# jmloveyj/ros_navigation

Measured on AMD Instinct MI355X. Metric: replan cycles/sec (HIMM+VFH++A*) on 4096x4096 grid, higher is better.
Workload: dtype int32; 1 GPU; full replan loop on 4096x4096 f32 grid (res 0.05 m); one step = one turn of the 20-stage A* pipeline = 20 passes of [100032-ray HIMM batch + fused compose -> 256 VFH+ poses -> 256 grid-A* queries (one launch)]; 30% rectangle obstacles (seed 2); 4 ray batches / pose sets / query sets in rotation; cycles_per_pass=256, rays_per_pass=100032, rotating_input_sets=4, astar_queries_checked=15360, astar_queries_answered=15360, astar_bucket_width=128000, astar_pipeline_depth=20, parallelism=query-sharded x1, full=False

## Files before the change

ros_navigation_amd/csrc/astar.hip:

```cpp
#include "engine.hpp"

#include <algorithm>
#include <cfloat>
#include <cmath>
#include <cstdlib>
#include <cstring>
#include <chrono>
#include <thread>
#include <vector>

using namespace rna;

namespace {

constexpr int COST_D = 1414;

struct HostTrace {
  bool on = getenv("RNA_HOST_TRACE") != nullptr;
  double us[8] = {};
  long n = 0, queries = 0;
  std::chrono::steady_clock::time_point t;
  void start() { if (on) t = std::chrono::steady_clock::now(); }
  void lap(int k) {
    if (!on) return;
// ... 166 lines not shown
  static const bool nowait = getenv("RNA_ASTAR_NOWAIT") != nullptr;
  static const int per_look = getenv("RNA_ASTAR_QUERIES_PER_LOOK") ? std::max(1, atoi(getenv("RNA_ASTAR_QUERIES_PER_LOOK"))) : 3;
  int slot = -1;
  for (int spin = 0; slot < 0; ++spin) {
    int oldest = 0;
    for (int d = 0; d < a.depth; ++d) {
      if (a.stage[d].seq < a.stage[oldest].seq) oldest = d;
      if (!a.stage[d].busy && (slot < 0 || a.stage[d].seq < a.stage[slot].seq)) slot = d;
    }
    if (slot < 0) {
      int order[AstarDevice::MAX_DEPTH], nb = 0;
      for (int d = 0; d < a.depth; ++d) if (a.stage[d].busy) order[nb++] = d;
      std::sort(order, order + nb, [&](int x, int y) { return a.stage[x].seq < a.stage[y].seq; });
      const int ask = (spin & 7) == 7 ? nb : std::min(nb, per_look);
      for (int k = 0; k < ask && slot < 0; ++k) {
        const int d = order[k];
        g_trace.queries += 1;
        if (hipEventQuery(a.stage[d].done) != hipSuccess) { (void)hipGetLastError(); continue; }
        bool sent = false;
        RNA_TRY(stage_settled(e, d, &sent));
        if (sent) continue;
        a.stage[d].busy = false;
        slot = d;
        if (g_trace.on && g_stage.armed[d]) {
          float f = 0;
          if (hipEventElapsedTime(&f, g_stage.a[d], g_stage.c[d]) == hipSuccess) {
            g_stage.gpu_ms += f; g_stage.n += 1;
            g_stage.host_busy_ms += std::chrono::duration<double, std::milli>(std::chrono::steady_clock::now() - g_stage.t_enq[d]).count();
          }
          g_stage.armed[d] = false;
        }
      }
    }
    if (slot >= 0) break;
    if (nowait) { slot = oldest; break; }
    static const int wait_us = getenv("RNA_ASTAR_WAIT_US") ? atoi(getenv("RNA_ASTAR_WAIT_US")) : 50;
    if (spin >= 2 && wait_us > 0) std::this_thread::sleep_for(std::chrono::microseconds(wait_us));
    else std::this_thread::yield();
  }
  g_trace.lap(0);
  const unsigned long long prev = a.launches + 1 >= (unsigned long long)a.ring_n ? a.launches + 1 - (unsigned long long)a.ring_n : 0;
  for (int d = 0; prev > 0 && d < a.depth; ++d)
    if (a.stage[d].busy && a.stage[d].seq == prev) RNA_TRY(stage_wait(e, d));
  *slot_out = slot;
  return RNA_OK;
}

int launch_chunk(rna_engine* e, const rna_astar_query* q_dev, int n, int32_t* paths_dev, int max_len,
                 rna_astar_result* res_dev, int* slot_out) {
  AstarDevice& a = e->astar;
  const bool pipelined = a.depth > 1;
  int slot = 0, r = -1;
  g_trace.start();
  if (pipelined) RNA_TRY(pick_stage(e, &slot));
  g_trace.lap(1);
  if (!pipelined && stage_pending(a, 0)) RNA_TRY(stage_wait(e, 0));
  AstarStage& s = a.stage[slot];
  hipStream_t search = stage_stream(e, slot), prep = search;
  if (pipelined) {
    if (s.busy) RNA_HIP(e, hipStreamWaitEvent(search, s.done, 0));
    if (g_trace.on) {
      if (!g_stage.a[slot]) { (void)hipEventCreate(&g_stage.a[slot]); (void)hipEventCreate(&g_stage.c[slot]); }
      (void)hipEventRecord(g_stage.a[slot], search);
      g_stage.t_enq[slot] = std::chrono::steady_clock::now();
    }
    r = (int)(a.launches % (unsigned long long)a.ring_n);
    RNA_TRY(side_stream(e, &prep));
    RNA_HIP(e, hipEventRecord(a.ev_init, e->stream));
    RNA_HIP(e, hipStreamWaitEvent(prep, a.ev_init, 0));
    if (a.ring[r].used) RNA_HIP(e, hipStreamWaitEvent(prep, a.ring[r].free, 0));
  }
  RNA_TRY(tsa_snapshot(e, slot, r, prep));
  if (pipelined) {
    RNA_HIP(e, hipEventRecord(s.snap_done, prep));
    s.snap_pending = true;
  }
  RNA_TRY(tsa_order(e, slot, r, prep, q_dev, n));
  if (pipelined) {
    RNA_HIP(e, hipEventRecord(a.ev_prep, prep));
    RNA_HIP(e, hipStreamWaitEvent(search, a.ev_prep, 0));
  }
  if (s.retry_flag) *s.retry_flag = 0;
  RNA_TRY(tsa_search(e, slot, r, search, q_dev, n, paths_dev, max_len, res_dev));
  if (s.retry_armed) RNA_HIP(e, hipMemcpyAsync(s.retry_flag, tsa_retry_count(e, slot), sizeof(int), hipMemcpyDeviceToHost, search));
  if (pipelined) {
    RNA_HIP(e, hipEventRecord(a.ring[r].free, search));
    a.ring[r].used = true;
    if (g_trace.on) { (void)hipEventRecord(g_stage.c[slot], search); g_stage.armed[slot] = true; }
  }
  g_trace.lap(2);
  if (pipelined) {
    RNA_HIP(e, hipEventRecord(s.done, search));
    s.busy = true;
  }
  a.launches += 1;
  s.seq = a.launches;
  a.last_queries = q_dev; a.last_results = res_dev; a.last_n = n; a.last_slot = slot;
  if (slot_out) *slot_out = slot;
  g_trace.lap(3);
  if (pipelined) g_trace.n += 1;
  return RNA_OK;
}

}

namespace rna {
#ifdef RNA_TSA_STATS
void tsa_stats_dump();
#endif
int astar_settle(rna_engine* e) {
  AstarDevice& a = e->astar;
  for (int d = 0; d < a.depth && d < AstarDevice::MAX_DEPTH; ++d)
    if (stage_pending(a, d)) RNA_TRY(stage_wait(e, d));
  return RNA_OK;
}
int astar_release(rna_engine* e) {
  AstarDevice& a = e->astar;
  (void)sync_all(e);
  stage_trace_dump();
  g_trace.dump();
#ifdef RNA_TSA_STATS
  tsa_stats_dump();
#endif
  for (AstarStage& s : a.stage) free_stage(s);
  if (a.ev_init) { (void)hipEventDestroy(a.ev_init); a.ev_init = nullptr; }
  if (a.ev_prep) { (void)hipEventDestroy(a.ev_prep); a.ev_prep = nullptr; }
  for (AstarRingEntry& r : a.ring) {
    if (r.free) (void)hipEventDestroy(r.free);
    r = AstarRingEntry{};
  }
  dev_free(&a.ring_mem);
  a.ring_n = 0;
  if (a.retry_flag) { (void)hipHostFree(a.retry_flag); a.retry_flag = nullptr; }
  dev_free(&a.queries_dev); dev_free(&a.results_dev); dev_free(&a.paths_dev);
  a.paths_cap = 0;
  a.last_queries = nullptr; a.last_results = nullptr; a.last_n = 0;
  return RNA_OK;
}
}

extern "C" int rna_astar_configure(rna_engine* e, int max_queries, int queue_capacity, int bucket_width) {
  if (!e || max_queries < 0 || queue_capacity < 0 || bucket_width < 0) return RNA_EINVAL;
  if (bucket_width != 0 && bucket_width < 2 * COST_D) return fail(e, RNA_EINVAL, "bucket_width must be >= 2828");
  RNA_ENTER(e);
  RNA_HIP(e, hipStreamSynchronize(e->stream));
  AstarDevice& a = e->astar;
  if (max_queries || queue_capacity) astar_release(e);
  if (const char* d = getenv("RNA_ASTAR_PIPELINE")) {
    const int dd = atoi(d);
    if (dd >= 1 && dd != a.depth) { astar_release(e); a.depth = dd; }
  }
  if (max_queries) a.max_queries = max_queries;
  if (bucket_width) a.bucket_width = bucket_width;
  return RNA_OK;
}

extern "C" int rna_astar_set_pipeline_depth(rna_engine* e, int depth) {
  if (!e || depth < 1 || depth > AstarDevice::MAX_DEPTH) return RNA_EINVAL;
  RNA_ENTER(e);
  if (depth != e->astar.depth) {
    astar_release(e);
    e->astar.depth = depth;
  }
  char advice[448];
  if (rna_hw_queue_advice(depth, advice, sizeof(advice))) e->err = advice;
  return RNA_OK;
}
// ... 108 lines not shown
```

ros_navigation_amd/csrc/astar_tile.hip:

```cpp
#include "engine.hpp"
#include <algorithm>
#include <cstring>
#include <vector>

using namespace rna;

namespace rna {

constexpr int TI = 64, TJ = 16;
constexpr int TILE_WORDS = TI * TJ;
constexpr int AUX_WORDS = 64;
constexpr int MASK_STRIDE = TILE_WORDS + 32 + 128;
constexpr int TSA_WAVES = 8;
constexpr int TSA_WAVES_PER_EU = 8;
constexpr int TSA_HPASS = 4;
constexpr int TSA_IDLE_SLEEP = 4;
constexpr int TSA_PRIO_FIRST = 0;
constexpr int TSA_BT_PRIO = 3;
constexpr int TSA_SCOPE = __HIP_MEMORY_SCOPE_AGENT;
constexpr int TSA_MAX_TILE_WORDS = 2048;
constexpr int COST_S = 1000, COST_D = 1414;
constexpr int INF = 0x7fffffff;
constexpr int KU = 0x40000000;
constexpr int SCR_CNT = 84 + 192 + 48 + 64;
// ... 868 lines not shown
        cp[0] = make_uint4((unsigned)pp0, (unsigned)pp1, (unsigned)pp2, (unsigned)pp3);
        cp[1] = make_uint4((unsigned)pp4, (unsigned)pp5, (unsigned)pp6, (unsigned)pp7);
        cp[2] = make_uint4((unsigned)pp8, (unsigned)pp9, (unsigned)pp10, (unsigned)pp11);
        cp[3] = make_uint4((unsigned)pp12, (unsigned)pp13, (unsigned)pp14, (unsigned)pp15);
      }
      __builtin_amdgcn_wave_barrier();
      const int xl_ = lane & 31;
      const bool xr_ = lane >= 32;
      const int v_ = (xl_ >= 1 && xl_ <= TJ) ? (int)scr[276 + (lane & 32) + xl_ - 1] : 0;
      const int xv = (int)scr[84 + 128 + lane];
      const unsigned eb_ = scr[84 + 192 + 48 + lane];
      const int vs_ = v_ & -(int)((eb_ >> (xr_ ? 4 : 3)) & 1u), vu_ = v_ & -(int)((eb_ >> (xr_ ? 2 : 0)) & 1u), vd_ = v_ & -(int)((eb_ >> (xr_ ? 7 : 5)) & 1u);
      const int from_below_ = lane_p1(vu_) + nD, from_above_ = lane_m1(vd_) + nD;
      const int ux_ = max3i(vs_ + nS, from_below_, from_above_);
      const bool imp = (xl_ <= TJ + 1) & (ux_ > xv);
      const unsigned long long im = __builtin_amdgcn_ballot_w64(imp);
      const unsigned lo = (unsigned)im, hi = (unsigned)(im >> 32);
      colw = (lo & 1u) | ((lo >> 12) & 32u) | ((hi & 1u) << 2) | ((hi >> 10) & 128u) | ((lo & 0x1fffeu) ? 8u : 0u) | ((hi & 0x1fffeu) ? 16u : 0u);
      if (im) {
        const int hX_ = tsa_octile24(xr_ ? i0 + TI : i0 - 1, j0 + xl_ - 1, gi, gj);
        wave_halves_max_i32(imp ? ux_ - hX_ : (int)0x80000000, kfW, kfE);
      }
      __builtin_amdgcn_wave_barrier();
    }
    const unsigned am = colw | (wakeN ? 2u : 0u) | (wakeS ? 64u : 0u);
    const unsigned wm = am & (unsigned)__builtin_amdgcn_ballot_w64(nb_t >= 0);
    if (wm) {
      asm volatile("s_waitcnt vmcnt(0)" ::: "memory");
      int kf = __builtin_amdgcn_inverse_ballot_w64(0x29ull) ? kfW : kfE;
      kf = __builtin_amdgcn_inverse_ballot_w64(0x02ull) ? kfN : kf;
      kf = __builtin_amdgcn_inverse_ballot_w64(0x40ull) ? kfS : kf;
      int key = (key_base - kf) >> key_shift;
      key = key < 0 ? 0 : (key > TSA_NCLS - 1 ? TSA_NCLS - 1 : key);
      TSA_T(t_w1);
      sch.wake8(__builtin_amdgcn_inverse_ballot_w64((unsigned long long)wm), nb_t, (unsigned)key, lane, spare);
      TSA_T(t_w2);
      TSA_ACC(3, t_w1, t_w2);
      TSA_CNT(13, 1);
    }
  }
  asm volatile("; TSA_MARK job_end");
  TSA_T(t_d);
  TSA_ACC(2, t_c, t_d);
  TSA_ACC(6, t_w0, t_d);
  if (lane_in == 0) { atomicAdd(&scr[SCR_CNT], (unsigned)__builtin_popcount(rowchg)); atomicAdd(&scr[SCR_CNT + 1], 1u); }
  }
tsa_job_done:
  asm volatile("s_waitcnt vmcnt(0)" ::: "memory");
  {
    int t_f = t_in;
    asm volatile("" : "+s"(t_f));
    const int again = sch.finish(t_f, lane_in, spare, scr + SCR_CNT);
    if (!again) break;
    first_w = again >> 1;
    sticky_w = 1;
    TSA_CNT(7, 1);
    TSA_CNT(22, 1);
  }
  }
#undef TSA_ROW_CHANGED
#undef TSA_H
}

struct TsaLaunch {
  int rows, cols, tiles_i, tiles_j, s0, s1;
  const rna_astar_query* queries;
  TsaStage S;
  int bucket_width;
  int prio_first;
  int retry, n;
  int* retry_count;
  int* retry_list;
  int retry_base;
  TsaStage S2;
  int32_t* paths;
  int max_path_len;
  int32_t* rev_all;
  int rev_cap;
  rna_astar_result* results;
};
constexpr int TSA_FOUND = -1000;

constexpr int BW = TI + 2;
__device__ __forceinline__ void tsa_backtrace_wave(const TsaLaunch& A, const TsaStage& S, const int sl, const int q, const rna_astar_result r,
                                                   const int lane, unsigned* s_tile, unsigned char* s_mask) {
  const int rows = A.rows, cols = A.cols, tiles_i = A.tiles_i, tiles_j = A.tiles_j;
  const int ncell = rows * cols, ntile = tiles_i * tiles_j;
  const unsigned* tmap = S.tmap + (size_t)sl * ntile;
  const size_t page_base = (size_t)sl * ((size_t)S.cap + 1);
  const int start = tsa_unwrap_lin(A.queries[q].start, rows, cols, A.s0, A.s1);
  const int goal = tsa_unwrap_lin(A.queries[q].goal, rows, cols, A.s0, A.s1);
  const int si = start % rows, sj = start / rows;
  int ci = goal % rows, cj = goal / rows;
  int* rev = A.rev_all + (size_t)q * A.rev_cap;
  const int k = lane & 7;
  const int wk = (k == 1 || k == 3 || k == 4 || k == 6) ? COST_S : COST_D;
  const int di = kdi_of(k), dj = kdj_of(k);
  const int off = di + dj * BW;
  int len = 0;
  bool ok = true, done = false;
#ifdef RNA_TSA_STATS
  unsigned long long bt_loads = 0, bt_load_ticks = 0;
#endif
  while (ok && !done) {
#ifdef RNA_TSA_STATS
    const unsigned long long t_l0 = wall_clock64();
#endif
    const int ti = ci >> 6, tj = cj >> 4;
    const int t = tj * tiles_i + ti;
    unsigned pgl = 0u;
    {
      const int nti = lane < 8 ? ti + di : ti, ntj = lane < 8 ? tj + dj : tj;
      if (lane < 9 && nti >= 0 && ntj >= 0 && nti < tiles_i && ntj < tiles_j) pgl = ld_l2(&tmap[ntj * tiles_i + nti]);
    }
    auto gpage = [&](int src) -> size_t {
      const unsigned lp = (unsigned)__shfl((int)pgl, src);
      return page_base + lp;
    };
    {
      const int xl = lane & 31;
      const bool xr = lane >= 32;
      const unsigned* pown = S.pages + (gpage(8) << 10);
      const unsigned top = ld_l2(&S.pages[(gpage(1) << 10) + (TJ - 1) * TI + lane]);
      const unsigned bot = ld_l2(&S.pages[(gpage(6) << 10) + lane]);
      const int xdir = xl == 0 ? (xr ? 2 : 0) : (xl <= TJ ? (xr ? 4 : 3) : (xr ? 7 : 5));
      const int xrow = xl == 0 ? TJ - 1 : (xl <= TJ ? xl - 1 : 0);
      const size_t gpx = gpage(xdir);
      unsigned X = 0u;
      if (xl <= TJ + 1) X = ld_l2(&S.paux[gpx * AUX_WORDS + (xr ? 0 : 16) + xrow]);
      unsigned tv[TJ];
#pragma unroll
      for (int b = 0; b < TJ; ++b) tv[b] = ld_l2(&pown[b * TI + lane]);
      const uint4 mv = *reinterpret_cast<const uint4*>(S.nbr_tm + (size_t)t * MASK_STRIDE + lane * 16);
      __builtin_amdgcn_wave_barrier();
      s_tile[lane + 1] = top;
      s_tile[(TJ + 1) * BW + lane + 1] = bot;
      if (xl <= TJ + 1) s_tile[xl * BW + (xr ? TI + 1 : 0)] = X;
#pragma unroll
      for (int b = 0; b < TJ; ++b) s_tile[(b + 1) * BW + lane + 1] = tv[b];
      *reinterpret_cast<uint4*>(&s_mask[lane * 16]) = mv;
    }
    asm volatile("s_waitcnt vmcnt(0) lgkmcnt(0)" ::: "memory");
    __builtin_amdgcn_wave_barrier();
#ifdef RNA_TSA_STATS
    bt_loads += 1; bt_load_ticks += wall_clock64() - t_l0;
#endif
    int il = ci & (TI - 1), jl = cj & (TJ - 1);
    unsigned uc = s_tile[(jl + 1) * BW + il + 1];
    for (;;) {
      if (lane == 0 && len < A.rev_cap) rev[len] = cj * rows + ci;
      ++len;
      if (ci == si && cj == sj) { done = true; break; }
      if (len > ncell || uc == 0u) { ok = false; break; }
      const unsigned mc = s_mask[il * 16 + jl];
      const unsigned un = s_tile[(jl + 1) * BW + il + 1 + off];
      const bool hit = (lane < 8) & (((mc >> k) & 1u) != 0u) & (un != 0u) & (un == uc + (unsigned)wk);
      const unsigned long long m = __ballot(hit);
      if (!m) { ok = false; break; }
      const int src = __builtin_ctz((unsigned)m);
      uc = (unsigned)__builtin_amdgcn_readlane((int)un, src);
      const int sdi = kdi_of(src), sdj = kdj_of(src);
      ci += sdi; cj += sdj; il += sdi; jl += sdj;
      if (il < 0 || jl < 0 || il >= TI || jl >= TJ) break;
    }
  }
#ifdef RNA_TSA_STATS
  if (lane == 0) { atomicAdd(&g_tsa_stat[27], bt_loads); atomicAdd(&g_tsa_stat[28], bt_load_ticks); atomicAdd(&g_tsa_stat[29], (unsigned long long)len); }
#endif
  if (!ok) {
    if (lane == 0) A.results[q] = rna_astar_result{1, 0, INF, r.expanded, r.rounds, r.buckets};
    return;
  }
  if (len > A.max_path_len || len > A.rev_cap) {
    if (lane == 0) A.results[q] = rna_astar_result{3, len, r.cost, r.expanded, r.rounds, r.buckets};
    return;
  }
  asm volatile("s_waitcnt vmcnt(0)" ::: "memory");
  __builtin_amdgcn_wave_barrier();
  int32_t* path = A.paths + (size_t)q * A.max_path_len;
  for (int i = lane; i < len; i += 64) path[i] = tsa_buffer_lin(rev[len - 1 - i], rows, cols, A.s0, A.s1);
  if (lane == 0) A.results[q] = rna_astar_result{0, len, r.cost, r.expanded, r.rounds, r.buckets};
}

template <int WAVES, bool RETRY>
__global__ void __launch_bounds__(WAVES * 64) __attribute__((amdgpu_waves_per_eu(TSA_WAVES_PER_EU, TSA_WAVES_PER_EU))) tsa_search_kernel(const TsaLaunch A) {
  constexpr int TSA_THREADS = WAVES * 64;
  __shared__ __attribute__((aligned(16))) unsigned s_scr[WAVES][SCR_WORDS];
  extern __shared__ unsigned s_dyn[];
  __shared__ __attribute__((aligned(16))) unsigned s_node[TSA_NP];
  __shared__ __attribute__((aligned(16))) unsigned s_head[TSA_NCLS];
  __shared__ unsigned s_bm[TSA_BMW];
  __shared__ unsigned s_qc[TSA_QC];
  __shared__ int s_best, s_state, s_bucket, s_bucket0, s_jobs_done, s_jobs_noop, s_jobs_sticky, s_expanded, s_nalloc, s_any;
  __shared__ int s_count, s_spill, s_idle, s_open_left, s_open_pos, s_reruns;

  __shared__ int s_q, s_rank;
  if (!RETRY) {
    if (threadIdx.x == 0) { const int k = atomicAdd(A.S.ticket, 1); s_rank = k; s_q = A.S.perm[k]; }
  } else {
    if (threadIdx.x == 0) { s_q = A.retry_list[A.retry_base + (int)blockIdx.x]; s_rank = 1 << 30; }
  }
  __syncthreads();
  const int q = __builtin_amdgcn_readfirstlane(s_q);
  if (q < 0) return;
  if (RETRY && threadIdx.x == 0) A.S2.ticket[8 + blockIdx.x] = q;
  const TsaStage& S = RETRY ? A.S2 : A.S;
  const int sl = RETRY ? (int)blockIdx.x : q;
  if (__builtin_amdgcn_readfirstlane(s_rank) < A.prio_first) __builtin_amdgcn_s_setprio(3);
  const int tid = threadIdx.x, lane = tid & 63, wv = __builtin_amdgcn_readfirstlane(tid >> 6);
#ifdef RNA_TSA_STATS
  const unsigned long long t_kernel0 = wall_clock64();
#endif
  const int rows = A.rows, cols = A.cols, tiles_i = A.tiles_i, tiles_j = A.tiles_j;
  rna_astar_query qu = A.queries[q];
  const int ncell = rows * cols;
  const int ntile = tiles_i * tiles_j;
  const int nt_words = (ntile + 31) >> 5;
  unsigned* const s_st2 = s_dyn;
  unsigned* const s_open = s_dyn + 2 * nt_words;
  unsigned* const s_far = s_dyn + 3 * nt_words;
  rna_astar_result* const results = A.results;

  const bool valid = qu.start >= 0 && qu.goal >= 0 && qu.start < ncell && qu.goal < ncell;
  if (!valid) {
    if (tid == 0) results[q] = rna_astar_result{2, 0, INF, 0, 0, 0};
    return;
  }
  qu.start = tsa_unwrap_lin(qu.start, rows, cols, A.s0, A.s1);
  qu.goal = tsa_unwrap_lin(qu.goal, rows, cols, A.s0, A.s1);
  const int si = qu.start % rows, sj = qu.start / rows;
  const int gi = qu.goal % rows, gj = qu.goal / rows;

  TsaCtx C;
  C.rows = rows; C.cols = cols; C.tiles_i = tiles_i; C.tiles_j = tiles_j;
  C.tiles_magic = tiles_i > 1 ? (unsigned)(0x100000000ull / (unsigned)tiles_i) + 1u : 0u;
  C.pages = S.pages + (((size_t)sl * ((size_t)S.cap + 1)) << 10);
  C.paux = S.paux + (size_t)sl * ((size_t)S.cap + 1) * AUX_WORDS;
  C.tmap = S.tmap + (size_t)sl * ntile;
  C.owner = S.owner + (size_t)sl * (S.cap + 1);
  C.cap = S.cap;
  C.nalloc = &s_nalloc;
  C.nbr_tm = S.nbr_tm;
  C.gi = gi; C.gj = gj;
  C.ts = tile_of(si, sj, tiles_i); C.sa = si & (TI - 1); C.sb = sj & (TJ - 1);
  C.tg = tile_of(gi, gj, tiles_i); C.ga = gi & (TI - 1); C.gb = gj & (TJ - 1);

  for (int w = tid; w < 4 * nt_words; w += TSA_THREADS) s_dyn[w] = 0u;
  for (int w = tid; w < TSA_NCLS; w += TSA_THREADS) s_head[w] = 0xffffu;
  for (int w = tid; w < TSA_BMW; w += TSA_THREADS) s_bm[w] = 0xffffffffu;
  for (int w = tid; w < TSA_QC; w += TSA_THREADS) s_qc[w] = 0xffffffffu;
  if (lane >= 48) s_scr[wv][68 + lane - 48] = 0u;
  if (lane < 4) s_scr[wv][SCR_CNT + lane] = 0u;
  {
    const unsigned ms = C.nbr_tm[(size_t)C.ts * MASK_STRIDE + C.sa * 16 + C.sb], mg = C.nbr_tm[(size_t)C.tg * MASK_STRIDE + C.ga * 16 + C.gb];
    if (qu.goal != qu.start && (mg == 0u || ms == 0u)) {
      if (tid == 0) results[q] = rna_astar_result{1, 0, INF, 0, 0, 0};
      return;
    }
  }
  {
    const int used_raw = S.nalloc[sl];
    const int used = used_raw < C.cap ? used_raw : C.cap;
    if (used > 0) {
      for (int p = 1 + tid; p <= used; p += TSA_THREADS) C.tmap[C.owner[p]] = 0u;
      asm volatile("s_waitcnt vmcnt(0)" ::: "memory");
// ... 96 lines not shown
          if (r == 1 && open_left > 0 && ((atomicAnd(&s_open[tt >> 5], ~(1u << (tt & 31))) >> (tt & 31)) & 1u)) {
            atomicSub(&s_open_left, 1);
            atomicSub(&s_count, 1);
            r = 2;
          }
        }
        r = __builtin_amdgcn_readfirstlane(r);
        if (r <= 0) continue;
        t = tt;
        first = r >> 1;
      }
      TSA_T(t_p1);
      TSA_ACC(4, t_p0, t_p1);
      TSA_CNT(7, 1);
      tsa_job(sch, s_scr[wv], lane, t, C, first, bucket_end_u, key_base, key_shift, &spare TSA_ACC_ARG);
      idle = false;
      open_blocked = false;
    }
    __syncthreads();
    if (s_state >= 4) break;
    int tid_r = threadIdx.x;
    asm volatile("" : "+v"(tid_r));
    const bool spilled = s_spill != 0;
    __syncthreads();
    if (tid_r == 0) {
      if (!spilled && s_best != INF && (long long)s_best < bucket_end) s_state = 1;
      if (spilled) s_reruns += 1;
      s_any = 0; s_spill = 0; s_idle = 0; s_open_pos = 0;
    }
    __syncthreads();
    if (s_state == 1) break;
    int cnt = 0;
    for (int w = tid_r; w < nt_words; w += TSA_THREADS) {
      const unsigned b = s_far[w];
      s_open[w] = b;
      s_far[w] = 0u;
      cnt += __popc(b);
    }
    if (cnt) atomicAdd(&s_any, cnt);
    __syncthreads();
    if (tid_r == 0) {
      if (!s_any) s_state = (s_best != INF) ? 1 : 2;
      else { s_count = s_any; s_open_left = s_any; if (!spilled) s_bucket += 1; }
    }
    __syncthreads();
    if (s_state != 0) break;
  }
  if (lane == 0) {
    atomicAdd(&s_expanded, (int)s_scr[wv][SCR_CNT] * TI);
    atomicAdd(&s_jobs_done, (int)s_scr[wv][SCR_CNT + 2]);
    atomicAdd(&s_jobs_noop, (int)(s_scr[wv][SCR_CNT + 2] - s_scr[wv][SCR_CNT + 1]));
    atomicAdd(&s_jobs_sticky, (int)s_scr[wv][SCR_CNT + 3]);
  }
  __syncthreads();
  if (tid == 0) {
    unsigned long long* const cnt = tsa_counters_of(S);
    atomicAdd(&cnt[0], 1ull);
    atomicAdd(&cnt[1], (unsigned long long)s_nalloc);
    atomicAdd(&cnt[2], (unsigned long long)s_jobs_done);
    atomicAdd(&cnt[3], (unsigned long long)s_jobs_noop);
    atomicAdd(&cnt[4], (unsigned long long)s_jobs_sticky);
    atomicAdd(&cnt[5], (unsigned long long)(s_expanded / TI));
    atomicAdd(&cnt[6], (unsigned long long)(s_bucket - s_bucket0 + 1));
    if (s_reruns) atomicAdd(&cnt[7], (unsigned long long)s_reruns);
  }
#ifdef RNA_TSA_STATS
  tsa_acc[5] = wall_clock64() - t_life0;
  tsa_acc[12] = __builtin_amdgcn_s_memtime() - c_life0;
  if (lane == 0) for (int k = 0; k < 16; ++k) atomicAdd(&g_tsa_stat[k], tsa_acc[k]);
  if (lane == 0) for (int k = 18; k < 24; ++k) atomicAdd(&g_tsa_stat[k], tsa_acc[k]);
  if (tid == 0) { atomicAdd(&g_tsa_stat[16], (unsigned long long)s_nalloc); atomicAdd(&g_tsa_stat[17], 1ull); }
#endif
  if (tid == 0) S.nalloc[sl] = s_nalloc < C.cap ? s_nalloc : C.cap;
  const int state = s_state;
  const rna_astar_result r{state == 1 ? TSA_FOUND : (state >= 4 ? state : 1), 0, state == 1 ? s_best : INF, s_expanded,
                           (s_jobs_done + WAVES - 1) / WAVES, s_bucket - s_bucket0 + 1};
  if (state != 1) {
    if (tid == 0) {
      results[q] = r;
      if (!RETRY && state == 5 && A.retry_count) A.retry_list[atomicAdd(A.retry_count, 1)] = q;
    }
    return;
  }
  __syncthreads();
  if (wv != 0) return;
  asm volatile("s_waitcnt vmcnt(0)" ::: "memory");
  __builtin_amdgcn_s_setprio(TSA_BT_PRIO);
#ifdef RNA_TSA_STATS
  const unsigned long long t_bt0 = wall_clock64();
#endif
  tsa_backtrace_wave(A, S, sl, q, r, lane, s_node, reinterpret_cast<unsigned char*>(s_node + BW * (TJ + 2)));
#ifdef RNA_TSA_STATS
  if (lane == 0) { atomicAdd(&g_tsa_stat[24], wall_clock64() - t_bt0); atomicAdd(&g_tsa_stat[25], 1ull); atomicAdd(&g_tsa_stat[26], wall_clock64() - t_kernel0); }
#endif
}

__global__ void tsa_settled_kernel(int rows, int cols, int tiles_i, int tiles_j, const rna_astar_query* __restrict__ queries,
                                   const rna_astar_result* __restrict__ results, TsaStage S_main, TsaStage S_retry, const int* __restrict__ served,
                                   const int* __restrict__ retry_list, int n_retried, int32_t* __restrict__ counts, int s0, int s1) {
  __shared__ int s_cnt;
  const int q = blockIdx.x;
  int sl = q;
  bool retried = false;
  if (served)
    for (int r = 0; r < TSA_RETRY; ++r)
      if (served[r] == q) { sl = r; retried = true; }
  if (!retried)
    for (int r = 0; r < n_retried; ++r)
      if (retry_list[r] == q) { if (threadIdx.x == 0) counts[q] = -1; return; }
  const TsaStage& S = retried ? S_retry : S_main;
  if (threadIdx.x == 0) s_cnt = 0;
  __syncthreads();
  const rna_astar_result r = results[q];
  int cnt = 0;
  if (r.status == 0 || r.status == 3) {
    const int goal = tsa_unwrap_lin(queries[q].goal, rows, cols, s0, s1);
    const int gi = goal % rows, gj = goal / rows;
    const int used = S.nalloc[sl];
    for (size_t w = threadIdx.x; w < ((size_t)used << 10); w += blockDim.x) {
      const int p = 1 + (int)(w >> 10), l = (int)(w & 1023);
      const int t = (int)S.owner[(size_t)sl * (S.cap + 1) + p];
      const int i = (t % tiles_i) * TI + (l & (TI - 1)), j = (t / tiles_i) * TJ + (l >> 6);
      const unsigned u = S.pages[(((size_t)sl * ((size_t)S.cap + 1) + p) << 10) + l];
      if (u != 0u && i < rows && j < cols && (KU - (int)u) + tsa_octile(i, j, gi, gj) <= r.cost) ++cnt;
    }
  }
  atomicAdd(&s_cnt, cnt);
  __syncthreads();
  if (threadIdx.x == 0) counts[q] = s_cnt;
}

static inline int tsa_ntile(const rna_engine* e) {
  return ((e->geom.size[0] + TI - 1) / TI) * ((e->geom.size[1] + TJ - 1) / TJ);
}
bool tsa_supported(const rna_engine* e) { return (size_t)tsa_ntile(e) <= (size_t)TSA_MAX_TILE_WORDS * 32; }
int tsa_tiles(const rna_engine* e) { return tsa_ntile(e); }
size_t tsa_pool_bytes(int max_queries, int cap) { return (size_t)max_queries * ((size_t)cap + 1) * (TILE_WORDS + AUX_WORDS) * sizeof(unsigned); }
size_t tsa_retry_pool_bytes(const rna_engine* e) { return tsa_pool_bytes(TSA_RETRY, tsa_ntile(e)); }

constexpr size_t TSA_HEAD = 256, TSA_HEAD_SERVED = 8 * sizeof(int), TSA_HEAD_COUNT = TSA_HEAD_SERVED + TSA_RETRY * sizeof(int),
                 TSA_HEAD_COUNTERS = TSA_HEAD - TSA_COUNTER_WORDS * sizeof(unsigned long long);
static_assert(TSA_HEAD_COUNT + sizeof(int) <= TSA_HEAD_COUNTERS, "the two halves of a block's head do not overlap");
struct TsaCursor {
  size_t at = TSA_HEAD;
  size_t take(size_t bytes) { const size_t o = at; at += tsa_align256(bytes); return o; }
};
struct TsaStageBlock { size_t nalloc, perm, nbr_tm, tmap, owner, total; };
static TsaStageBlock tsa_stage_block(const rna_engine* e) {
  const size_t nq = (size_t)e->astar.max_queries, ntile = (size_t)tsa_ntile(e), cap = (size_t)e->astar.page_cap;
  TsaCursor c;
  return {c.take(nq * sizeof(int)), c.take(nq * sizeof(int)), c.take(ntile * MASK_STRIDE), c.take(nq * ntile * sizeof(unsigned)),
          c.take(nq * (cap + 1) * sizeof(unsigned)), c.at};
}
struct TsaRetryBlock { size_t nalloc, tmap, owner, list, total; };
static TsaRetryBlock tsa_retry_block(const rna_engine* e) {
  const size_t nq = (size_t)e->astar.max_queries, ntile = (size_t)tsa_ntile(e);
  TsaCursor c;
  return {c.take(TSA_RETRY * sizeof(int)), c.take(TSA_RETRY * ntile * sizeof(unsigned)), c.take(TSA_RETRY * (ntile + 1) * sizeof(unsigned)),
          c.take(nq * sizeof(int)), c.at};
}
struct TsaRingBlock { size_t perm, nbr_tm, total; };
static TsaRingBlock tsa_ring_block(const rna_engine* e) {
  TsaCursor c;
  return {c.take((size_t)e->astar.max_queries * sizeof(int)), c.take((size_t)tsa_ntile(e) * MASK_STRIDE), c.at};
}
size_t tsa_stage_bytes(const rna_engine* e) { return tsa_stage_block(e).total; }
size_t tsa_retry_bytes(const rna_engine* e) { return tsa_retry_block(e).total; }
size_t tsa_ring_bytes(const rna_engine* e) { return tsa_ring_block(e).total; }
template <typename T>
static T* tsa_at(char* block, size_t offset) { return reinterpret_cast<T*>(block + offset); }

static TsaStage tsa_stage_view(const rna_engine* e, int d) {
  const AstarDevice& a = e->astar;
  const AstarStage& s = a.stage[d];
  const TsaStageBlock L = tsa_stage_block(e);
  TsaStage S;
  S.cap = a.page_cap;
// ... 33 lines not shown
}
static int* tsa_retry_served(const rna_engine* e, int d) { char* b = e->astar.stage[d].retry_block; return b ? tsa_at<int>(b, TSA_HEAD_SERVED) : nullptr; }
int* tsa_retry_count(const rna_engine* e, int d) { char* b = e->astar.stage[d].retry_block; return b ? tsa_at<int>(b, TSA_HEAD_COUNT) : nullptr; }
static int* tsa_retry_list(const rna_engine* e, int d) { char* b = e->astar.stage[d].retry_block; return b ? tsa_at<int>(b, tsa_retry_block(e).list) : nullptr; }

int tsa_retry_prepare(rna_engine* e, int slot) {
  const TsaStage S = tsa_retry_view(e, slot, tsa_stage_view(e, slot));
  hipLaunchKernelGGL(tsa_zero_page0_kernel, dim3(TSA_RETRY), dim3(256), 0, e->stream, S.pages, S.paux, S.cap);
  RNA_HIP(e, hipGetLastError());
  return RNA_OK;
}
int tsa_stage_prepare(rna_engine* e, int slot) {
  const TsaStage S = tsa_stage_view(e, slot);
  hipLaunchKernelGGL(tsa_zero_page0_kernel, dim3(e->astar.max_queries), dim3(256), 0, e->stream, S.pages, S.paux, S.cap);
  RNA_HIP(e, hipGetLastError());
  return RNA_OK;
}

static_assert(sizeof(TsaLaunch) <= sizeof(AstarStage::last_launch), "AstarStage::last_launch holds a TsaLaunch");

int tsa_retry_launch(rna_engine* e, int d, hipStream_t st, int count) {
  const AstarStage& s = e->astar.stage[d];
  TsaLaunch A;
  memcpy(&A, s.last_launch, sizeof(A));
  A.retry = 1;
  A.retry_count = nullptr;
  A.S2 = tsa_retry_view(e, d, A.S);
  for (int base = 0; base < count; base += TSA_RETRY) {
    A.retry_base = base;
    const int wgs = std::min(TSA_RETRY, count - base);
    if (e->astar.depth > 1) hipLaunchKernelGGL((tsa_search_kernel<TSA_WAVES, true>), dim3(wgs), dim3(TSA_WAVES * 64), s.last_lds, st, A);
    else hipLaunchKernelGGL((tsa_search_kernel<16, true>), dim3(wgs), dim3(16 * 64), s.last_lds, st, A);
    RNA_HIP(e, hipGetLastError());
  }
  return RNA_OK;
}

struct TsaGrid { int rows, cols, ti, tj; };
static TsaGrid tsa_grid(const rna_engine* e) {
  const int rows = e->geom.size[0], cols = e->geom.size[1];
  return {rows, cols, (rows + TI - 1) / TI, (cols + TJ - 1) / TJ};
}
int tsa_snapshot(rna_engine* e, int d, int ring, hipStream_t st) {
  const TsaGrid G = tsa_grid(e);
  KernelTimer kt(e, RNA_K_ASTAR_INIT, st);
  hipLaunchKernelGGL(tsa_snapshot_kernel, dim3(std::min(G.ti * G.tj, 4096)), dim3(256), 0, st, e->nbr, G.rows, G.cols, G.ti, G.tj,
                     tsa_launch_view(e, d, ring).nbr_tm, e->geom.start[0], e->geom.start[1]);
  RNA_HIP(e, hipGetLastError());
  return RNA_OK;
}
int tsa_order(rna_engine* e, int d, int ring, hipStream_t st, const rna_astar_query* q_dev, int n) {
  const TsaGrid G = tsa_grid(e);
  KernelTimer kt(e, RNA_K_ASTAR_RESET, st);
  const int ranked = n <= 2048 ? 1 : 0;
  hipLaunchKernelGGL(tsa_prepare_kernel, dim3(1), dim3(256), ranked ? (size_t)n * sizeof(int) : 0, st, tsa_launch_view(e, d, ring), q_dev, n, G.rows,
                     G.cols, ranked, tsa_retry_served(e, d));
  RNA_HIP(e, hipGetLastError());
  return RNA_OK;
}
int tsa_search(rna_engine* e, int d, int ring, hipStream_t st, const rna_astar_query* q_dev, int n, int32_t* paths_dev, int max_len,
               rna_astar_result* res_dev) {
  AstarDevice& a = e->astar;
  AstarStage& s = a.stage[d];
  const TsaGrid G = tsa_grid(e);
  const TsaStage S = tsa_launch_view(e, d, ring);
  KernelTimer kt(e, RNA_K_ASTAR_SEARCH, st);
  const size_t nt_bytes = (size_t)((G.ti * G.tj + 31) / 32) * sizeof(unsigned);
  TsaLaunch A;
  memset(&A, 0, sizeof(A));
  A.rows = G.rows; A.cols = G.cols; A.tiles_i = G.ti; A.tiles_j = G.tj; A.s0 = e->geom.start[0]; A.s1 = e->geom.start[1];
  A.queries = q_dev; A.S = S; A.bucket_width = a.bucket_width; A.paths = paths_dev; A.max_path_len = max_len;
  A.rev_all = s.rev; A.rev_cap = a.rev_cap; A.results = res_dev;
  A.retry = 0; A.n = n; A.S2 = S;
  A.prio_first = a.depth > 1 ? TSA_PRIO_FIRST : 0;
  if (const char* pf = getenv("RNA_TSA_PRIO_FIRST")) A.prio_first = atoi(pf);
  size_t lds_dyn = 4 * nt_bytes;
  if (const char* pad = getenv("RNA_TSA_LDS_PAD")) lds_dyn += (size_t)atoi(pad);
  const bool can_retry = s.retry_flag != nullptr;
  A.retry_count = can_retry ? tsa_retry_count(e, d) : nullptr;
  A.retry_list = can_retry ? tsa_retry_list(e, d) : nullptr;
  A.retry_base = 0;
  static const bool wide_env = getenv("RNA_TSA_WIDE") != nullptr;
  const bool wide = wide_env || n <= 32;
  if (a.depth > 1 && !wide) hipLaunchKernelGGL((tsa_search_kernel<TSA_WAVES, false>), dim3(n), dim3(TSA_WAVES * 64), lds_dyn, st, A);
  else hipLaunchKernelGGL((tsa_search_kernel<16, false>), dim3(n), dim3(16 * 64), lds_dyn, st, A);
  RNA_HIP(e, hipGetLastError());
  memcpy(s.last_launch, &A, sizeof(A));
  s.last_lds = lds_dyn;
  s.last_retried = 0;
  s.retry_armed = can_retry;
  return RNA_OK;
}

int tsa_counters_read(rna_engine* e, unsigned long long* out, bool reset) {
  AstarDevice& a = e->astar;
  for (int k = 0; k < TSA_COUNTER_WORDS; ++k) out[k] = 0ull;
  for (int d = 0; d < AstarDevice::MAX_DEPTH; ++d) {
    for (int view = 0; view < 2; ++view) {
      char* base = view ? a.stage[d].retry_block : a.stage[d].block;
      if (!base) continue;
      unsigned long long w[TSA_COUNTER_WORDS];
      char* cnt = base + TSA_HEAD_COUNTERS;
      RNA_HIP(e, hipMemcpyAsync(w, cnt, sizeof(w), hipMemcpyDeviceToHost, e->stream));
      if (reset) RNA_HIP(e, hipMemsetAsync(cnt, 0, sizeof(w), e->stream));
      RNA_HIP(e, hipStreamSynchronize(e->stream));
      for (int k = 0; k < TSA_COUNTER_WORDS; ++k) out[k] += w[k];
    }
  }
  return RNA_OK;
}

#ifdef RNA_TSA_STATS
void tsa_stats_dump() {
  unsigned long long st[32];
  if (hipMemcpyFromSymbol(st, HIP_SYMBOL(g_tsa_stat), sizeof(st)) != hipSuccess) return;
  const double jobs = (double)st[7];
  if (jobs <= 0) return;
  const double busy = (double)(st[0] + st[1] + st[2]);
  fprintf(stderr, "[tsa stats] per job us: loads issued + arrived %.2f (of load+halo), wake tests + queueing %.2f of which queueing %.2f (of results); jobs that queue wake-ups %.1f%%; a job that finds nothing %.2f us\n",
          st[9] * 0.01 / jobs, st[6] * 0.01 / jobs, st[3] * 0.01 / jobs, 100.0 * (double)st[13] / jobs, st[15] * 0.01 / (double)std::max<unsigned long long>(1, st[10]));
  fprintf(stderr, "[tsa stats] searches %.0f, tiles touched %.0f (%.1f per search), jobs per touched tile %.2f, jobs that find nothing %.3f of all\n", (double)st[17],
          (double)st[16], (double)st[16] / (double)std::max<unsigned long long>(1, st[17]), jobs / (double)std::max<unsigned long long>(1, st[16]), (double)st[10] / jobs);
  fprintf(stderr, "[tsa stats, tile kernel, all launches] jobs %.0f (%.1f%% no-op) | per job us: load+halo %.2f sweeps %.2f results %.2f | wave lifetime %.1f wave-ms, in jobs %.1f wave-ms (%.1f%%), taking jobs %.1f wave-ms (%.1f%%) | row evaluations per job %.1f, extra horizontal passes %.1f | shader clock while searching %.0f MHz\n",
          jobs, 100.0 * (double)st[10] / jobs, st[0] * 0.01 / jobs, st[1] * 0.01 / jobs, st[2] * 0.01 / jobs, st[5] * 1e-5, busy * 1e-5,
          100.0 * busy / (double)st[5], st[4] * 1e-5, 100.0 * (double)st[4] / (double)st[5], st[8] / jobs, st[11] / jobs,
          100.0 * (double)st[12] / (double)std::max<unsigned long long>(1, st[5]));
  if (st[25]) fprintf(stderr, "[tsa stats] backtrace (one wavefront, the workgroup's LDS held meanwhile): %.1f us per found path, %.1f %% of the workgroup's residence (%.2f ms from its first instruction to the end of the backtrace, found paths only)\n",
                      st[24] * 0.01 / (double)st[25], 100.0 * (double)st[24] / (double)std::max<unsigned long long>(1, st[26]), st[26] * 1e-5 / (double)st[25]);
  if (st[25]) fprintf(stderr, "[tsa stats] backtrace: %.0f cells and %.1f tile loads per path (%.1f cells per load), a tile load %.2f us (%.0f %% of the backtrace), a step %.3f us\n",
                      (double)st[29] / (double)st[25], (double)st[27] / (double)st[25], (double)st[29] / (double)std::max<unsigned long long>(1, st[27]),
                      st[28] * 0.01 / (double)std::max<unsigned long long>(1, st[27]), 100.0 * (double)st[28] / (double)std::max<unsigned long long>(1, st[24]),
                      (double)(st[24] - st[28]) * 0.01 / (double)std::max<unsigned long long>(1, st[29]));
  fprintf(stderr, "[tsa stats] sticky turns (the wavefront kept a tile that was woken while it ran) %.3f of all jobs, of which %.3f find nothing\n",
          (double)st[22] / jobs, (double)st[23] / (double)std::max<unsigned long long>(1, st[22]));
  fprintf(stderr, "[tsa stats] first jobs (a tile's first in a bucket: the rows a new bound releases, and what they flag) %.3f of all, %.1f row evaluations and %.1f changed rows each; rows changed per job %.1f; rows sent to the scan per job %.2f\n",
          (double)st[18] / jobs, (double)st[19] / (double)std::max<unsigned long long>(1, st[18]), (double)st[20] / (double)std::max<unsigned long long>(1, st[18]), (double)st[21] / jobs, (double)st[14] / jobs);
}
#endif

int tsa_settled(rna_engine* e, int slot, const rna_astar_query* q, const rna_astar_result* r, int n, int32_t* d_counts) {
  const TsaGrid G = tsa_grid(e);
  const TsaStage S = tsa_stage_view(e, slot);
  const AstarStage& s = e->astar.stage[slot];
  hipLaunchKernelGGL(tsa_settled_kernel, dim3(n), dim3(1024), 0, e->stream, G.rows, G.cols, G.ti, G.tj, q, r, S,
                     s.retry_pool ? tsa_retry_view(e, slot, S) : S, tsa_retry_served(e, slot), tsa_retry_list(e, slot),
                     s.retry_pool ? s.last_retried : 0, d_counts, e->geom.start[0], e->geom.start[1]);
  RNA_HIP(e, hipGetLastError());
  return RNA_OK;
}

}
```

Baseline: 173,200 replan cycles/s.

## Split A* path backtrace into a separate trace kernel with eight paths per block

In the pipelined throughput configuration, the search kernel no longer runs the path backtrace itself. It writes a provisional found result and exits, so its 8-wave block frees its CU and LDS sooner. A new trace kernel then runs one wave per found query, eight per block, each with its own LDS image. The retry-count readback is moved after the search launch so it runs before the trace kernel. The cost is an extra kernel launch and re-reading results and tile maps from global memory.

```diff
diff --git a/ros_navigation_amd/csrc/astar.hip b/ros_navigation_amd/csrc/astar.hip
--- a/ros_navigation_amd/csrc/astar.hip
+++ b/ros_navigation_amd/csrc/astar.hip
@@ -272,7 +272,6 @@
   }
   if (s.retry_flag) *s.retry_flag = 0;
   RNA_TRY(tsa_search(e, slot, r, search, q_dev, n, paths_dev, max_len, res_dev));
-  if (s.retry_armed) RNA_HIP(e, hipMemcpyAsync(s.retry_flag, tsa_retry_count(e, slot), sizeof(int), hipMemcpyDeviceToHost, search));
   if (pipelined) {
     RNA_HIP(e, hipEventRecord(a.ring[r].free, search));
     a.ring[r].used = true;
diff --git a/ros_navigation_amd/csrc/astar_tile.hip b/ros_navigation_amd/csrc/astar_tile.hip
--- a/ros_navigation_amd/csrc/astar_tile.hip
+++ b/ros_navigation_amd/csrc/astar_tile.hip
@@ -974,6 +974,8 @@
 constexpr int TSA_FOUND = -1000;
 
 constexpr int BW = TI + 2;
+constexpr int TSA_TRACE_IMAGE_WORDS = BW * (TJ + 2) + TILE_WORDS / 4;
+static_assert((BW * (TJ + 2)) % 4 == 0 && TSA_TRACE_IMAGE_WORDS % 4 == 0, "the masks of an image, and the next image, start on 16 bytes");
 __device__ __forceinline__ void tsa_backtrace_wave(const TsaLaunch& A, const TsaStage& S, const int sl, const int q, const rna_astar_result r,
                                                    const int lane, unsigned* s_tile, unsigned char* s_mask) {
   const int rows = A.rows, cols = A.cols, tiles_i = A.tiles_i, tiles_j = A.tiles_j;
@@ -991,6 +993,7 @@
   const int off = di + dj * BW;
   int len = 0;
   bool ok = true, done = false;
+  asm volatile("; TSA_WALK begin");
 #ifdef RNA_TSA_STATS
   unsigned long long bt_loads = 0, bt_load_ticks = 0;
 #endif
@@ -1073,6 +1076,8 @@
   for (int i = lane; i < len; i += 64) path[i] = tsa_buffer_lin(rev[len - 1 - i], rows, cols, A.s0, A.s1);
   if (lane == 0) A.results[q] = rna_astar_result{0, len, r.cost, r.expanded, r.rounds, r.buckets};
 }
+
+__host__ __device__ constexpr bool tsa_trace_inside(int waves, bool retry) { return retry || waves != TSA_WAVES; }
 
 template <int WAVES, bool RETRY>
 __global__ void __launch_bounds__(WAVES * 64) __attribute__((amdgpu_waves_per_eu(TSA_WAVES_PER_EU, TSA_WAVES_PER_EU))) tsa_search_kernel(const TsaLaunch A) {
@@ -1335,17 +1340,38 @@
     }
     return;
   }
-  __syncthreads();
-  if (wv != 0) return;
-  asm volatile("s_waitcnt vmcnt(0)" ::: "memory");
+  if constexpr (!tsa_trace_inside(WAVES, RETRY)) {
+    if (tid == 0) {
+      results[q] = rna_astar_result{0, 0, r.cost, r.expanded, r.rounds, r.buckets};
+      asm volatile("s_waitcnt vmcnt(0)" ::: "memory");
+    }
+  } else {
+    __syncthreads();
+    if (wv != 0) return;
+    asm volatile("s_waitcnt vmcnt(0)" ::: "memory");
+    __builtin_amdgcn_s_setprio(TSA_BT_PRIO);
+#ifdef RNA_TSA_STATS
+    const unsigned long long t_bt0 = wall_clock64();
+#endif
+    tsa_backtrace_wave(A, S, sl, q, r, lane, s_node, reinterpret_cast<unsigned char*>(s_node + BW * (TJ + 2)));
+#ifdef RNA_TSA_STATS
+    if (lane == 0) { atomicAdd(&g_tsa_stat[24], wall_clock64() - t_bt0); atomicAdd(&g_tsa_stat[25], 1ull); atomicAdd(&g_tsa_stat[26], wall_clock64() - t_kernel0); }
+#endif
+  }
+}
+
+constexpr int TSA_TRACE_PATHS = 8;
+__global__ void __launch_bounds__(TSA_TRACE_PATHS * 64) __attribute__((amdgpu_waves_per_eu(TSA_WAVES_PER_EU, TSA_WAVES_PER_EU))) tsa_trace_kernel(const TsaLaunch A) {
+  extern __shared__ __attribute__((aligned(16))) unsigned s_image[];
+  const int lane = threadIdx.x & 63, wv = __builtin_amdgcn_readfirstlane(threadIdx.x >> 6);
+  const int rank = (int)blockIdx.x * TSA_TRACE_PATHS + wv;
+  if (rank >= A.n) return;
+  const int q = __builtin_amdgcn_readfirstlane(A.S.perm[rank]);
+  const rna_astar_result r = A.results[q];
+  if (r.status != 0 || r.path_len != 0) return;
   __builtin_amdgcn_s_setprio(TSA_BT_PRIO);
-#ifdef RNA_TSA_STATS
-  const unsigned long long t_bt0 = wall_clock64();
-#endif
-  tsa_backtrace_wave(A, S, sl, q, r, lane, s_node, reinterpret_cast<unsigned char*>(s_node + BW * (TJ + 2)));
-#ifdef RNA_TSA_STATS
-  if (lane == 0) { atomicAdd(&g_tsa_stat[24], wall_clock64() - t_bt0); atomicAdd(&g_tsa_stat[25], 1ull); atomicAdd(&g_tsa_stat[26], wall_clock64() - t_kernel0); }
-#endif
+  unsigned* const s_tile = s_image + wv * TSA_TRACE_IMAGE_WORDS;
+  tsa_backtrace_wave(A, A.S, q, q, r, lane, s_tile, reinterpret_cast<unsigned char*>(s_tile + BW * (TJ + 2)));
 }
 
 __global__ void tsa_settled_kernel(int rows, int cols, int tiles_i, int tiles_j, const rna_astar_query* __restrict__ queries,
@@ -1545,9 +1571,16 @@
   A.retry_base = 0;
   static const bool wide_env = getenv("RNA_TSA_WIDE") != nullptr;
   const bool wide = wide_env || n <= 32;
-  if (a.depth > 1 && !wide) hipLaunchKernelGGL((tsa_search_kernel<TSA_WAVES, false>), dim3(n), dim3(TSA_WAVES * 64), lds_dyn, st, A);
+  const bool throughput = a.depth > 1 && !wide;
+  if (throughput) hipLaunchKernelGGL((tsa_search_kernel<TSA_WAVES, false>), dim3(n), dim3(TSA_WAVES * 64), lds_dyn, st, A);
   else hipLaunchKernelGGL((tsa_search_kernel<16, false>), dim3(n), dim3(16 * 64), lds_dyn, st, A);
   RNA_HIP(e, hipGetLastError());
+  if (can_retry) RNA_HIP(e, hipMemcpyAsync(s.retry_flag, A.retry_count, sizeof(int), hipMemcpyDeviceToHost, st));
+  if (throughput && !tsa_trace_inside(TSA_WAVES, false)) {
+    hipLaunchKernelGGL(tsa_trace_kernel, dim3((n + TSA_TRACE_PATHS - 1) / TSA_TRACE_PATHS), dim3(TSA_TRACE_PATHS * 64),
+                       (size_t)TSA_TRACE_PATHS * TSA_TRACE_IMAGE_WORDS * sizeof(unsigned), st, A);
+    RNA_HIP(e, hipGetLastError());
+  }
   memcpy(s.last_launch, &A, sizeof(A));
   s.last_lds = lds_dyn;
   s.last_retried = 0;
```

Result: faster. 182,200 replan cycles/s, median of 6 (+5.2%).
